# PaulTFLi/Machine-Learning-Replications

Measured on AMD Instinct MI355X. Metric: train_rows_per_sec, higher is better.
Workload: dtype fp32

## Files before the change

machine-learning-replications_amd/ops/csrc/svm_ws.hip:

```cpp
#include <type_traits>

#include "common.h"

namespace hfens {

struct WsProb {
  long long zoff;
  long long aoff;
  int l;
  int npos;
  double Cp, Cn;
  float ngl2e;
  int pad;
};

struct WsState {
  int done;
  int outer;
  long long inner;
  double gap;
  int nc;
  int nws;
  int nprev;
  int pad;
// ... 119 lines not shown
    if (pos ? a < C : a > 0) { su = -yg; ku = ws_key(su); }
    if (pos ? a > 0 : a < C) { sl = yg; kl = ws_key(sl); }
    X.keys[P.aoff + t] = ku;
    X.keys[X.n + P.aoff + t] = kl;
  }
  su = wave_max_f64_exact(su);
  sl = wave_max_f64_exact(sl);
  if ((threadIdx.x & 63) == 0) {
    if (su > -kWsInf) atomicMax(&X.gkey[2 * b], f64_okey(su));
    if (sl > -kWsInf) atomicMax(&X.gkey[2 * b + 1], f64_okey(sl));
  }
}

__global__ __launch_bounds__(256) void ws_init_kernel(const WsProb* __restrict__ probs, const float* __restrict__ zcat,
                                                      int F, float* __restrict__ zn, double* __restrict__ alpha,
                                                      double* __restrict__ G, WsState* __restrict__ states,
                                                      WsAux X) {
  const int b = blockIdx.y;
  const WsProb P = probs[b];
  const int t = blockIdx.x * blockDim.x + threadIdx.x;
  if (blockIdx.x * blockDim.x >= P.l) return;
  if (blockIdx.x == 0 && threadIdx.x == 0) states[b] = WsState{0, 0, 0, 0.0, 0, 0, 0, 0, 0, 0, 0, 0, 0, 0};
  const bool valid = t < P.l;
  if (valid) {
    const float* z = zcat + (P.zoff + t) * F;
    float s = 0.f;
    for (int k = 0; k < F; ++k) s = fmaf(z[k], z[k], s);
    zn[P.aoff + t] = s;
    alpha[P.aoff + t] = 0.0;
    G[P.aoff + t] = -1.0;
  }
  ws_publish_keys(P, b, t, valid, 0.0, -1.0, X);
}

constexpr size_t ws_sel_lds_bytes(int Q) { return 32 * 4 + 4096 * 4 + 1024 * 4 + (size_t)Q * 4; }

template <int M, typename Emit>
__device__ __forceinline__ int ws_pick_lists(const unsigned (&ku)[M], const unsigned (&kl)[M], int t0, int k_up,
                                             int k_low, int* shi, int* binfo, int* hist, Emit emit) {
  const int tid = threadIdx.x;
  for (int i = tid; i < 4096; i += kWsThreads) hist[i] = 0;
  if (tid < 8) binfo[tid] = 0;
  __syncthreads();
#pragma unroll
  for (int m = 0; m < M; ++m) {
    hist_add(hist, ku[m] != 0u, (int)(ku[m] >> 21));
    hist_add(hist, kl[m] != 0u, 2048 + (int)(kl[m] >> 21));
  }
  __syncthreads();
  ws_find_bin(hist, k_up, k_low, shi, binfo);
  __syncthreads();
  const unsigned bu1 = binfo[0], bl1 = binfo[2];
  const int au1 = binfo[1], al1 = binfo[3];
  for (int i = tid; i < 4096; i += kWsThreads) hist[i] = 0;
  __syncthreads();
#pragma unroll
  for (int m = 0; m < M; ++m) {
    hist_add(hist, ku[m] != 0u && (ku[m] >> 21) == bu1, (int)((ku[m] >> 10) & 2047));
    hist_add(hist, kl[m] != 0u && (kl[m] >> 21) == bl1, 2048 + (int)((kl[m] >> 10) & 2047));
  }
  __syncthreads();
  ws_find_bin(hist, k_up - au1, k_low - al1, shi, binfo + 4);
  __syncthreads();
  const unsigned Tu = (bu1 << 11) | (unsigned)binfo[4], Tl = (bl1 << 11) | (unsigned)binfo[6];
  const int need_u = k_up - au1 - binfo[5], need_l = k_low - al1 - binfo[7];
  unsigned selm = 0u;
  int base = 0;
#pragma unroll
  for (int side = 0; side < 2; ++side) {
    const unsigned T = side ? Tl : Tu;
    const int need = side ? need_l : need_u;
    int wt = 0;
#pragma unroll
    for (int m = 0; m < M; ++m) {
      const unsigned k = side ? kl[m] : ku[m];
      wt += __popcll(__ballot(k && (k >> 10) == T && !((selm >> m) & 1u)));
    }
    int ttot;
    int trank = wave_base(wt, shi, &ttot);
    unsigned pick = 0u;
    int ws_cnt = 0;
#pragma unroll
    for (int m = 0; m < M; ++m) {
      const unsigned k = side ? kl[m] : ku[m];
      const bool cand = k && !((selm >> m) & 1u);
      const bool tie = cand && (k >> 10) == T;
      const unsigned long long tb = __ballot(tie);
      const bool take = cand && ((k >> 10) > T || (tie && trank + __popcll(tb & lanes_below()) < need));
      trank += __popcll(tb);
      if (take) pick |= 1u << m;
      ws_cnt += __popcll(__ballot(take));
    }
    int stot;
    int pos = base + wave_base(ws_cnt, shi, &stot);
#pragma unroll
    for (int m = 0; m < M; ++m) {
      const bool take = (pick >> m) & 1u;
      const unsigned long long tb = __ballot(take);
      if (take) emit(pos + __popcll(tb & lanes_below()), t0 + 64 * m);
      pos += __popcll(tb);
    }
    selm |= pick;
    base += stot;
  }
  return base;
}

struct WsCand {
  int* idx;
  unsigned* ku;
  unsigned* kl;
  int ncand;
};
constexpr int kWsCandM = 8;
constexpr int kWsCandBlk = kWsCandM * kWsThreads;

template <int M, int Q, bool kWriteIdx, bool kCand = false>
__device__ __forceinline__ int ws_select_body(const WsProb& P, int b, WsState* S, int* __restrict__ wsidx,
                                              int* __restrict__ wsprev, double eps, int max_outer, const WsAux& X,
                                              int* shi, int* binfo, int* hist, unsigned* bm, int* widx,
                                              const WsCand& C = WsCand{nullptr, nullptr, nullptr, 0}) {
  const int nprev = S->nprev;
  const int tid = threadIdx.x;
  const int lane = tid & 63, wave = tid >> 6;
  const int L = kCand ? C.ncand : P.l;
  const int t0 = wave * 64 * M + lane;
  const long long c0 = __builtin_amdgcn_s_memtime();
  const unsigned long long gku = X.gkey[2 * b], gkl = X.gkey[2 * b + 1];
  const double Gmax = gku ? f64_from_okey(gku) : -kWsInf;
  const double Gmax2 = gkl ? f64_from_okey(gkl) : -kWsInf;
  const double gap = Gmax + Gmax2;
  unsigned ku[M], kl[M];
  int nu = 0, nl = 0;
#pragma unroll
  for (int m = 0; m < M; ++m) {
    const int t = t0 + 64 * m;
    if (kCand) {
      ku[m] = t < L ? C.ku[(size_t)b * C.ncand + t] : 0u;
      kl[m] = t < L ? C.kl[(size_t)b * C.ncand + t] : 0u;
    } else {
      ku[m] = t < L ? __builtin_nontemporal_load(X.keys + P.aoff + t) : 0u;
      kl[m] = t < L ? __builtin_nontemporal_load(X.keys + X.n + P.aoff + t) : 0u;
    }
  }
#pragma unroll
  for (int m = 0; m < M; ++m) {
    nu += __popcll(__ballot(ku[m] != 0u));
    nl += __popcll(__ballot(kl[m] != 0u));
  }
  if (!kCand)
    for (int i = tid; i < 1024; i += kWsThreads) bm[i] = 0;
  int n_up;
  wave_base(nu | (nl << 16), shi, &n_up);
  const int n_low = n_up >> 16;
  n_up &= 0xFFFF;
  if (!(gap >= eps) || S->outer >= max_outer || n_up == 0 || n_low == 0) {
    if (tid == 0) { S->done = 1; S->gap = gap; S->nc = 0; S->nws = 0; }
    return -1;
  }
  if (tid == 0) { X.gkey[2 * b] = 0ull; X.gkey[2 * b + 1] = 0ull; }
  const int k_up = min(Q / 4, n_up), k_low = min(Q / 4, n_low);
  const long long c0a = __builtin_amdgcn_s_memtime();
  const int nnew = ws_pick_lists<M>(ku, kl, t0, k_up, k_low, shi, binfo, hist, [&](int i, int p) {
    if (kCand) {
      widx[i] = C.idx[(size_t)b * C.ncand + p];
    } else {
      widx[i] = p;
      atomicOr(&bm[p >> 5], 1u << (p & 31));
    }
  });
  const long long c0b = __builtin_amdgcn_s_memtime();
  const long long c0c = c0b;
  __syncthreads();
  const int pv = tid < nprev ? wsprev[(size_t)b * (Q / 2) + tid] : -1;
  bool again = false;
  if (pv >= 0) {
    if (kCand) {
      for (int w = 0; w < nnew; ++w) again |= widx[w] == pv;
    } else {
      again = (bm[pv >> 5] >> (pv & 31)) & 1u;
    }
  }
  const bool keep = pv >= 0 && !again;
  const unsigned long long kb = __ballot(keep);
  int ktot;
  const int kpos = nnew + wave_base(__popcll(kb), shi, &ktot) + __popcll(kb & lanes_below());
  if (keep) widx[kpos] = pv;
  __syncthreads();
  const int nws = nnew + ktot;
  for (int w = tid; w < nnew; w += kWsThreads) wsprev[(size_t)b * (Q / 2) + w] = widx[w];
  if (kWriteIdx)
    for (int w = tid; w < nws; w += kWsThreads) wsidx[(size_t)b * Q + w] = widx[w];
  const long long c1 = __builtin_amdgcn_s_memtime();
  if (tid == 0) {
    S->cyc_select += c1 - c0;
    S->cyc_p0 += c0a - c0;
    S->cyc_p1 += c0b - c0a;
    S->cyc_p2 += c0c - c0b;
    S->nws = nws;
    S->nprev = nnew;
    S->gap = gap;
  }
  return nws;
}

template <int Q>
__global__ __launch_bounds__(kWsThreads) void ws_cand_kernel(const WsProb* __restrict__ probs,
                                                             const WsState* __restrict__ states, WsAux X, WsCand C) {
  constexpr int M = kWsCandM;
  constexpr int per = Q / 2;
  const int b = blockIdx.y, blk = blockIdx.x;
  if (states[b].done) return;
  const WsProb P = probs[b];
  const int tid = threadIdx.x;
  const int lane = tid & 63, wave = tid >> 6;
  const int beg = blk * kWsCandBlk;
  int* out_idx = C.idx + (size_t)b * C.ncand + (size_t)blk * per;
  unsigned* out_ku = C.ku + (size_t)b * C.ncand + (size_t)blk * per;
  unsigned* out_kl = C.kl + (size_t)b * C.ncand + (size_t)blk * per;
  __shared__ int shi[16], binfo[16];
  __shared__ int hist[4096];
  __shared__ int pick[per];
  const int t0 = wave * 64 * M + lane;
  unsigned ku[M], kl[M];
  int nu = 0, nl = 0;
#pragma unroll
  for (int m = 0; m < M; ++m) {
    const int t = beg + t0 + 64 * m;
    ku[m] = t < P.l ? __builtin_nontemporal_load(X.keys + P.aoff + t) : 0u;
    kl[m] = t < P.l ? __builtin_nontemporal_load(X.keys + X.n + P.aoff + t) : 0u;
  }
#pragma unroll
  for (int m = 0; m < M; ++m) {
    nu += __popcll(__ballot(ku[m] != 0u));
    nl += __popcll(__ballot(kl[m] != 0u));
  }
  int n_up;
  wave_base(nu | (nl << 16), shi, &n_up);
  const int n_low = n_up >> 16;
  n_up &= 0xFFFF;
  const int np = (n_up == 0 && n_low == 0) ? 0
                 : ws_pick_lists<M>(ku, kl, t0, min(Q / 4, n_up), min(Q / 4, n_low), shi, binfo, hist,
                                    [&](int i, int p) { pick[i] = beg + p; });
  __syncthreads();
  if (tid < per) {
    const int t = tid < np ? pick[tid] : -1;
    out_idx[tid] = t;
    out_ku[tid] = t >= 0 ? X.keys[P.aoff + t] : 0u;
    out_kl[tid] = t >= 0 ? X.keys[X.n + P.aoff + t] : 0u;
  }
}

template <int M, int Q>
__global__ __launch_bounds__(kWsThreads) void ws_select_kernel(
    const WsProb* __restrict__ probs, WsState* __restrict__ states, int* __restrict__ wsidx,
    int* __restrict__ wsprev, double eps, int max_outer, WsAux X) {
  const int b = blockIdx.x;
  WsState* S = states + b;
  if (S->done) return;
  const WsProb P = probs[b];
  extern __shared__ __attribute__((aligned(16))) unsigned char ws_lds[];
  int* shi = reinterpret_cast<int*>(ws_lds);
  int* binfo = shi + 16;
  int* hist = shi + 32;
  unsigned* bm = reinterpret_cast<unsigned*>(hist + 4096);
  int* widx = reinterpret_cast<int*>(bm + 1024);
  ws_select_body<M, Q, true>(P, b, S, wsidx, wsprev, eps, max_outer, X, shi, binfo, hist, bm, widx);
}

constexpr size_t ws_solve_lds_bytes(int Q, int FP) {
  return 64 * 4 + (size_t)Q * FP * 4 + (size_t)Q * 4 * 2 + (size_t)6 * Q * 4;
}

template <int FP, int Q, int TH>
__global__ __launch_bounds__(TH) void ws_solve_kernel(
    const WsProb* __restrict__ probs, WsState* __restrict__ states, const float* __restrict__ zcat, int F,
    const float* __restrict__ zn_all, double* __restrict__ alpha_all, const double* __restrict__ G_all,
    const int* __restrict__ wsidx, float* __restrict__ wsz, float* __restrict__ wsn, float* __restrict__ wdc,
    int Fp2, double eps, int max_inner, double inner_frac, long long* __restrict__ prof) {
  static_assert(Q % TH == 0 && (Q & (Q - 1)) == 0 && TH % 64 == 0 && TH <= 512, "whole slots per thread");
  static_assert(FP % 4 == 0, "z rows are read as float4");
  constexpr int SL = Q / TH;
  static_assert(SL % 2 == 0, "slots go in pairs (packed f32 fma)");
  constexpr int NW = TH / 64;
  constexpr unsigned kIdx = Q - 1;
  const int b = blockIdx.x;
  WsState* S = states + b;
  if (S->done) return;
  const WsProb P = probs[b];
  const int nws = S->nws;
  const int tid = threadIdx.x;
  const int lane = tid & 63, wave = tid >> 6;
  extern __shared__ __attribute__((aligned(16))) unsigned char ws_lds[];
  unsigned* red = reinterpret_cast<unsigned*>(ws_lds);
  float* zB = reinterpret_cast<float*>(ws_lds + 64 * 4);
  float* snB = zB + (size_t)Q * FP;
  int* widx = reinterpret_cast<int*>(snB + Q);
  float* gl = reinterpret_cast<float*>(widx + Q);
  float* al = gl + 2 * Q;
  float* kil = al + 2 * Q;
  const double* Gp = G_all + P.aoff;
  double* ap = alpha_all + P.aoff;
  const long long c1 = __builtin_amdgcn_s_memtime();
  {
    int wi[SL];
#pragma unroll
    for (int m = 0; m < SL; ++m) {
      const int s = tid + TH * m;
      wi[m] = s < nws ? wsidx[(size_t)b * Q + s] : -1;
    }
    float zv[SL][FP];
    float znv[SL];
#pragma unroll
    for (int m = 0; m < SL; ++m) {
      const float* zrow = zcat + (P.zoff + (wi[m] < 0 ? 0 : wi[m])) * F;
#pragma unroll
      for (int k = 0; k < FP; ++k) zv[m][k] = (wi[m] >= 0 && k < F) ? zrow[k] : 0.f;
      znv[m] = wi[m] >= 0 ? zn_all[P.aoff + wi[m]] : 0.f;
    }
#pragma unroll
    for (int m = 0; m < SL; ++m) {
      const int s = tid + TH * m;
      widx[s] = wi[m] < 0 ? 0 : wi[m];
      snB[s] = P.ngl2e * znv[m];
#pragma unroll
      for (int k = 0; k < FP; k += 4)
        *reinterpret_cast<f32x4*>(&zB[s * FP + k]) = f32x4{zv[m][k], zv[m][k + 1], zv[m][k + 2], zv[m][k + 3]};
    }
  }
  __syncthreads();
  const long long c2 = __builtin_amdgcn_s_memtime();
  const long long r2 = __builtin_amdgcn_s_memrealtime();
  bool valid[SL], pos[SL];
  int tt[SL];
  float y[SL], Cw[SL], a[SL], yg[SL], sn[SL], tu[SL], tl[SL];
  double a0[SL];
  f32x2 zp[SL / 2][FP];
#pragma unroll
  for (int m = 0; m < SL; ++m) {
    const int s = tid + TH * m;
    valid[m] = s < nws;
    tt[m] = valid[m] ? widx[s] : 0;
    pos[m] = tt[m] < P.npos;
    y[m] = pos[m] ? 1.f : -1.f;
    Cw[m] = (float)(pos[m] ? P.Cp : P.Cn);
    tu[m] = valid[m] ? (pos[m] ? Cw[m] : 0.f) : -INFINITY;
    tl[m] = valid[m] ? (pos[m] ? 0.f : Cw[m]) : -INFINITY;
    a0[m] = valid[m] ? ap[tt[m]] : 0.0;
    a[m] = (float)a0[m];
    yg[m] = valid[m] ? y[m] * (float)Gp[tt[m]] : 0.f;
    sn[m] = valid[m] ? snB[s] : 0.f;
#pragma unroll
    for (int k = 0; k < FP; k += 4) {
      const f32x4 v = valid[m] ? *reinterpret_cast<const f32x4*>(&zB[s * FP + k]) : f32x4{0.f, 0.f, 0.f, 0.f};
#pragma unroll
      for (int q = 0; q < 4; ++q) zp[m / 2][k + q][m & 1] = v[q];
    }
  }
  const float k2c = -2.f * P.ngl2e;
  const float Cpf = (float)P.Cp, Cnf = (float)P.Cn;
  auto krow = [&](int r, float (&out)[SL]) {
    f32x2 d[SL / 2];
#pragma unroll
    for (int h = 0; h < SL / 2; ++h) d[h] = f32x2{0.f, 0.f};
#pragma unroll
    for (int k = 0; k < FP; k += 4) {
      const f32x4 v = *reinterpret_cast<const f32x4*>(&zB[r * FP + k]);
#pragma unroll
      for (int q = 0; q < 4; ++q) {
#pragma unroll
        for (int h = 0; h < SL / 2; ++h) d[h] = __builtin_elementwise_fma(f32x2{v[q], v[q]}, zp[h][k + q], d[h]);
      }
    }
    const float snr = snB[r];
#pragma unroll
    for (int m = 0; m < SL; ++m)
      out[m] = __builtin_amdgcn_exp2f(fminf(fmaf(k2c, d[m / 2][m & 1], snr + sn[m]), 0.f));
  };
  auto red4 = [&](const unsigned* r) {
    unsigned x = 0u;
#pragma unroll
    for (int w = 0; w < NW; w += 4) {
      const uint4 v = *reinterpret_cast<const uint4*>(r + w);
      x = max(max(x, max(v.x, v.y)), max(v.z, v.w));
    }
    return x;
  };
  float tol_in = -1.f;
  const float epsf = (float)eps;
#ifdef HFENS_WS_STAMPS
  const bool pf = prof != nullptr;
  long long ph[6] = {0, 0, 0, 0, 0, 0};
  long long tp = pf ? __builtin_amdgcn_s_memtime() : 0;
#define WS_STAMP(k)                                         \
  if (pf) {                                                 \
    const long long tn = __builtin_amdgcn_s_memtime();      \
    ph[k] += tn - tp;                                       \
    tp = tn;                                                \
  }
#else
  const bool pf = false;
  long long ph[6] = {0, 0, 0, 0, 0, 0};
#define WS_STAMP(k)
#endif
  int it = 0;
  auto pair = [&](auto parc) -> bool {
    constexpr int par = decltype(parc)::value;
    float* glp = gl + par * Q;
    float* alp = al + par * Q;
    float* kip = kil + par * Q;
    unsigned* r1 = red + (0 * 2 + par) * NW;
    unsigned* r3 = red + (1 * 2 + par) * NW;
    unsigned* r2 = red + (2 * 2 + par) * NW;
    unsigned* r4 = red + (3 * 2 + par) * NW;
    unsigned k1 = 0u, k3 = 0u, k4 = 0u;
    bool low[SL];
#pragma unroll
    for (int m = 0; m < SL; ++m) {
      const unsigned s = (unsigned)(tid + TH * m);
      glp[s] = yg[m];
      alp[s] = a[m];
      const float ya = y[m] * a[m];
      const bool up = ya < tu[m];
      low[m] = -ya < tl[m];
      const unsigned um = 0u - (unsigned)up, lm = 0u - (unsigned)low[m];
      const unsigned kv = f32_okey(-yg[m]) & um;
      k4 = max(k4, kv);
      k1 = max(k1, ((kv & ~kIdx) | s) & um);
      k3 = max(k3, f32_okey(yg[m]) & lm);
    }
    k1 = wave_max_u32(k1);
    k3 = wave_max_u32(k3);
    k4 = wave_max_u32(k4);
    if (lane == 0) { r1[wave] = k1; r3[wave] = k3; r4[wave] = k4; }
    WS_STAMP(0)
    __syncthreads();
    const unsigned K1 = __builtin_amdgcn_readfirstlane(red4(r1));
    const unsigned K3 = __builtin_amdgcn_readfirstlane(red4(r3));
    const unsigned K4 = __builtin_amdgcn_readfirstlane(red4(r4));
    if (K1 == 0u || K3 == 0u) return false;
    const int i = (int)(K1 & kIdx);
    const float ygi = glp[i];
    const bool ipos = widx[i] < P.npos;
    const float yi = ipos ? 1.f : -1.f;
    const float Gi = yi * ygi;
    const float GmaxB = -ygi;
    const float lgap = f32_from_okey(K4) + f32_from_okey(K3);
    if (tol_in < 0.f) tol_in = fmaxf(0.9999f * epsf, (float)inner_frac * lgap);
    if (lgap < tol_in) return false;
    WS_STAMP(1)
    float Ki[SL];
    krow(i, Ki);
    unsigned k2 = 0u;
#pragma unroll
    for (int m = 0; m < SL; ++m) {
      const unsigned s = (unsigned)(tid + TH * m);
      kip[s] = Ki[m];
      const float gd = GmaxB + yg[m];
      const float q0 = 2.f - 2.f * Ki[m];
      const float quad = q0 <= 0.f ? 1e-12f : q0;
      const unsigned ok = 0u - (unsigned)(low[m] & (gd > 0.f));
      k2 = max(k2, ((f32_okey(gd * gd * __builtin_amdgcn_rcpf(quad)) & ~kIdx) | s) & ok);
    }
    k2 = wave_max_u32(k2);
    if (lane == 0) r2[wave] = k2;
    WS_STAMP(2)
    __syncthreads();
    const unsigned K2 = __builtin_amdgcn_readfirstlane(red4(r2));
    if (K2 == 0u) return false;
    const int j = (int)(K2 & kIdx);
    const float ai_old = alp[i], aj_old = alp[j];
    const float Kij = kip[j];
    const bool jpos = widx[j] < P.npos;
    const float yj = jpos ? 1.f : -1.f;
    const float Gj = yj * glp[j];
    const float Ci = ipos ? Cpf : Cnf, Cj = jpos ? Cpf : Cnf;
    WS_STAMP(3)
    const float q0 = 2.f - 2.f * Kij;
    const float rq = __builtin_amdgcn_rcpf(q0 <= 0.f ? 1e-12f : q0);
    float ao, bo, as, bs;
    {
      const float delta = (-Gi - Gj) * rq;
      const float diff = ai_old - aj_old;
      ao = ai_old + delta;
      bo = aj_old + delta;
      const bool c1 = (diff > 0.f) & (bo < 0.f), c2 = !(diff > 0.f) & (ao < 0.f);
      ao = c1 ? diff : (c2 ? 0.f : ao);
      bo = c1 ? 0.f : (c2 ? -diff : bo);
      const bool c3 = (diff > Ci - Cj) & (ao > Ci), c4 = !(diff > Ci - Cj) & (bo > Cj);
      ao = c3 ? Ci : (c4 ? Cj + diff : ao);
      bo = c3 ? Ci - diff : (c4 ? Cj : bo);
    }
    {
      const float delta = (Gi - Gj) * rq;
      const float sum = ai_old + aj_old;
      as = ai_old - delta;
      bs = aj_old + delta;
      const bool c1 = (sum > Ci) & (as > Ci), c2 = !(sum > Ci) & (bs < 0.f);
      as = c1 ? Ci : (c2 ? sum : as);
      bs = c1 ? sum - Ci : (c2 ? 0.f : bs);
      const bool c3 = (sum > Cj) & (bs > Cj), c4 = !(sum > Cj) & (as < 0.f);
      as = c3 ? sum - Cj : (c4 ? 0.f : as);
      bs = c3 ? Cj : (c4 ? sum : bs);
    }
    const bool opp = ipos != jpos;
    const float ai = opp ? ao : as, aj = opp ? bo : bs;
    const float ci = yi * (ai - ai_old), cj = yj * (aj - aj_old);
    WS_STAMP(4)
    float Kj[SL];
    krow(j, Kj);
#pragma unroll
    for (int m = 0; m < SL; ++m) {
      const int s = tid + TH * m;
      a[m] = s == i ? ai : (s == j ? aj : a[m]);
      yg[m] += fmaf(Ki[m], ci, Kj[m] * cj);
    }
    WS_STAMP(5)
    ++it;
    return true;
  };
  while (it < max_inner && pair(std::integral_constant<int, 0>{}) && it < max_inner &&
         pair(std::integral_constant<int, 1>{})) {
  }
#undef WS_STAMP
  if (pf && tid == 0) {
#pragma unroll
    for (int k = 0; k < 6; ++k) prof[(size_t)b * 6 + k] += ph[k];
  }
  int nc = 0;
#pragma unroll
  for (int m = 0; m < SL; ++m) {
    const int s = tid + TH * m;
    double anew = a0[m];
    if (valid[m] && a[m] != (float)a0[m]) {
      const double C = pos[m] ? P.Cp : P.Cn;
      anew = a[m] <= 0.f ? 0.0 : (a[m] >= Cw[m] ? C : a0[m] + ((double)a[m] - (double)(float)a0[m]));
      anew = fmin(fmax(anew, 0.0), C);
    }
    const bool ch = valid[m] && anew != a0[m];
    const unsigned long long cm = __ballot(ch);
    __syncthreads();
    if (lane == 0) red[wave] = (unsigned)__popcll(cm);
    __syncthreads();
    int wb = 0, tot = 0;
#pragma unroll
    for (int w = 0; w < NW; ++w) {
      const int v = (int)red[w];
      wb += w < wave ? v : 0;
      tot += v;
    }
    const int cpos = nc + wb + __popcll(cm & lanes_below());
    if (ch) {
      ap[tt[m]] = anew;
      for (int k = 0; k < Fp2; ++k) wsz[((size_t)b * Fp2 + k) * Q + cpos] = k < F ? zB[s * FP + k] : 0.f;
      wsn[(size_t)b * Q + cpos] = sn[m];
      wdc[(size_t)b * Q + cpos] = (float)((double)y[m] * (anew - a0[m]));
    }
    nc += tot;
  }
  const int ncp = (nc + 31) & ~31;
  for (int p = nc + tid; p < ncp; p += TH) {
    for (int k = 0; k < Fp2; ++k) wsz[((size_t)b * Fp2 + k) * Q + p] = 0.f;
    wsn[(size_t)b * Q + p] = 0.f;
    wdc[(size_t)b * Q + p] = 0.f;
  }
  const long long c3 = __builtin_amdgcn_s_memtime();
  const long long r3 = __builtin_amdgcn_s_memrealtime();
  if (tid == 0) {
    S->cyc_build += c2 - c1;
    S->cyc_inner += c3 - c2;
    S->cyc_p2 += r3 - r2;
    if (it == 0 || nc == 0) S->done = 1;
    S->nc = nc;
    S->outer += 1;
    S->inner += it;
  }
}

__device__ __forceinline__ unsigned sel4u(const unsigned (&v)[4], int m) {
  const unsigned m0 = 0u - (unsigned)(m == 0), m1 = 0u - (unsigned)(m == 1);
  const unsigned m2 = 0u - (unsigned)(m == 2), m3 = 0u - (unsigned)(m == 3);
  return (v[0] & m0) | (v[1] & m1) | (v[2] & m2) | (v[3] & m3);
}

constexpr int kKcQ = 256;
constexpr int kKcQP = kKcQ + 1;
constexpr int kKcTri = kKcQ * (kKcQ + 1) / 2;
constexpr size_t kc_zbuf_bytes(int KS) {
  return (size_t)2 * KS * kKcQP * 4 > (4096 + 1024) * 4 ? (size_t)2 * KS * kKcQP * 4 : (4096 + 1024) * 4;
}
constexpr size_t kc_lds_bytes(int KS) { return 128 + 2 * kKcQ * 4 + (kc_zbuf_bytes(KS) + 15) / 16 * 16 + (size_t)kKcTri * 4; }
static_assert(kc_lds_bytes(12) <= 163840, "the K-cached round must fit the CU's 160 KiB of LDS");

__device__ __forceinline__ int kc_rowstart(int r) { return r * kKcQ - ((r * (r - 1)) >> 1); }

__device__ __forceinline__ float sel4(const float (&v)[4], int m) {
  const unsigned u[4] = {__float_as_uint(v[0]), __float_as_uint(v[1]), __float_as_uint(v[2]), __float_as_uint(v[3])};
  return __uint_as_float(sel4u(u, m));
}
__device__ __forceinline__ int sel4(const int (&v)[4], int m) {
  const unsigned u[4] = {(unsigned)v[0], (unsigned)v[1], (unsigned)v[2], (unsigned)v[3]};
  return (int)sel4u(u, m);
}
__device__ __forceinline__ float rdlane_f(float v, int l) { return __int_as_float(__builtin_amdgcn_readlane(__float_as_int(v), l)); }

template <int M, int KS, bool kCand, bool kStamp = false>
__global__ __launch_bounds__(kWsThreads) void ws_kc_round_kernel(
    const WsProb* __restrict__ probs, WsState* __restrict__ states, const float* __restrict__ zcat, int F,
    const float* __restrict__ zn_all, double* __restrict__ alpha_all, const double* __restrict__ G_all,
    int* __restrict__ wsprev, float* __restrict__ wsz, float* __restrict__ wsn, float* __restrict__ wdc,
    int Fp2, double eps, int max_outer, int max_inner, double inner_frac, WsAux X, WsCand C,
    long long* __restrict__ prof = nullptr) {
  constexpr int Q = kKcQ;
  constexpr int SL = Q / 64;
  constexpr unsigned kIdx = Q - 1;
  static_assert(SL == 4, "sel4 assumes four slots per lane");
  const int b = blockIdx.x;
  WsState* S = states + b;
  if (S->done) return;
  const WsProb P = probs[b];
  const int tid = threadIdx.x;
  const int lane = tid & 63, wave = tid >> 6;
  extern __shared__ __attribute__((aligned(16))) unsigned char ws_lds[];
  int* shi = reinterpret_cast<int*>(ws_lds);
  int* binfo = shi + 16;
  int* widx = shi + 32;
  float* snB = reinterpret_cast<float*>(widx + Q);
  float* zbuf = snB + Q;
  int* hist = reinterpret_cast<int*>(zbuf);
  unsigned* bm = reinterpret_cast<unsigned*>(hist + 4096);
  float* tri = zbuf + (kc_zbuf_bytes(KS) + 15) / 16 * 4;
  const int nws = ws_select_body<M, Q, false, kCand>(P, b, S, nullptr, wsprev, eps, max_outer, X, shi, binfo,
                                                     hist, bm, widx, C);
  if (nws < 0) return;
  const long long c1 = __builtin_amdgcn_s_memtime();
  for (int e = tid; e < 2 * KS * Q; e += kWsThreads) {
    const int k = e / Q, s = e - k * Q;
    zbuf[k * kKcQP + s] = (s < nws && k < F) ? zcat[(P.zoff + widx[s]) * F + k] : 0.f;
  }
  if (tid < Q) snB[tid] = tid < nws ? P.ngl2e * zn_all[P.aoff + widx[tid]] : 0.f;
  __syncthreads();
  {
    const int r32 = lane & 31, hi = lane >> 5;
    const float k2 = -2.f * P.ngl2e;
    for (int t = wave; t < 36; t += kWsWaves) {
      int ta = 0, rem = t;
      while (rem >= 8 - ta) { rem -= 8 - ta; ++ta; }
      const int tb = ta + rem;
      f32x16 A = {0.f};
#pragma unroll
      for (int q = 0; q < KS; ++q) {
        const float* zr = zbuf + (2 * q + hi) * kKcQP;
        A = __builtin_amdgcn_mfma_f32_32x32x2f32(zr[ta * 32 + r32], zr[tb * 32 + r32], A, 0, 0, 0);
      }
      const int col = tb * 32 + r32;
      const float snc = snB[col];
#pragma unroll
      for (int r = 0; r < 16; ++r) {
        const int row = ta * 32 + 8 * (r >> 2) + 4 * hi + (r & 3);
        const float kv = __builtin_amdgcn_exp2f(fminf(fmaf(k2, A[r], snB[row] + snc), 0.f));
        if (row <= col) tri[kc_rowstart(row) + col - row] = kv;
      }
    }
  }
  __syncthreads();
  const long long c2 = __builtin_amdgcn_s_memtime();
  if (wave != 0) return;
  const double* Gp = G_all + P.aoff;
  double* ap = alpha_all + P.aoff;
  bool valid[SL], pos[SL];
  int tt[SL], rb[SL];
  float y[SL], Cw[SL], a[SL], yg[SL], tu[SL], tl[SL];
  double a0[SL];
#pragma unroll
  for (int m = 0; m < SL; ++m) {
    const int s = 64 * m + lane;
    valid[m] = s < nws;
    tt[m] = valid[m] ? widx[s] : 0;
    pos[m] = tt[m] < P.npos;
    y[m] = pos[m] ? 1.f : -1.f;
    Cw[m] = (float)(pos[m] ? P.Cp : P.Cn);
    tu[m] = valid[m] ? (pos[m] ? Cw[m] : 0.f) : -INFINITY;
    tl[m] = valid[m] ? (pos[m] ? 0.f : Cw[m]) : -INFINITY;
    a0[m] = valid[m] ? ap[tt[m]] : 0.0;
    a[m] = (float)a0[m];
    yg[m] = valid[m] ? y[m] * (float)Gp[tt[m]] : 0.f;
    rb[m] = kc_rowstart(s) - s;
  }
  auto krow = [&](int r, float (&out)[SL]) {
    const int ra = kc_rowstart(r) - r;
#pragma unroll
    for (int m = 0; m < SL; ++m) {
      const int s = 64 * m + lane;
      out[m] = tri[s >= r ? ra + s : rb[m] + r];
    }
  };
  const float Cpf = (float)P.Cp, Cnf = (float)P.Cn;
  const float epsf = (float)eps;
  float tol_in = -1.f;
  int it = 0;
  long long ph[5] = {0, 0, 0, 0, 0};
  long long tp = kStamp ? (long long)__builtin_amdgcn_s_memtime() : 0;
  auto stamp = [&](int k) {
    if constexpr (kStamp) {
      const long long tn = __builtin_amdgcn_s_memtime();
      ph[k] += tn - tp;
      tp = tn;
    }
  };
  while (it < max_inner) {
    unsigned k1 = 0u, k3 = 0u;
    bool low[SL];
#pragma unroll
    for (int m = 0; m < SL; ++m) {
      const unsigned s = (unsigned)(64 * m + lane);
      const float ya = y[m] * a[m];
      const bool up = ya < tu[m];
      low[m] = -ya < tl[m];
      const unsigned um = 0u - (unsigned)up, lm = 0u - (unsigned)low[m];
      k1 = max(k1, ((f32_okey(-yg[m]) & ~kIdx) | s) & um);
      k3 = max(k3, f32_okey(yg[m]) & lm);
    }
    const unsigned K1 = __builtin_amdgcn_readfirstlane(wave_max_u32(k1));
    const unsigned K3 = __builtin_amdgcn_readfirstlane(wave_max_u32(k3));
    stamp(0);
    if (K1 == 0u || K3 == 0u) break;
    const int i = (int)(K1 & kIdx), mi = i >> 6, li = i & 63;
    const float ygi = rdlane_f(sel4(yg, mi), li);
    const float ai_old = rdlane_f(sel4(a, mi), li);
    const bool ipos = __builtin_amdgcn_readlane(sel4(tt, mi), li) < P.npos;
    const float yi = ipos ? 1.f : -1.f;
    const float Gi = yi * ygi;
    const float GmaxB = -ygi;
    const float lgap = GmaxB + f32_from_okey(K3);
    if (tol_in < 0.f) tol_in = fmaxf(0.9999f * epsf, (float)inner_frac * lgap);
    if (lgap < tol_in) break;
    float Ki[SL];
    krow(i, Ki);
    stamp(1);
    unsigned k2 = 0u;
#pragma unroll
    for (int m = 0; m < SL; ++m) {
      const unsigned s = (unsigned)(64 * m + lane);
      const float gd = GmaxB + yg[m];
      const float q0 = 2.f - 2.f * Ki[m];
      const float quad = q0 <= 0.f ? 1e-12f : q0;
      const unsigned ok = 0u - (unsigned)(low[m] & (gd > 0.f));
      k2 = max(k2, ((f32_okey(gd * gd * __builtin_amdgcn_rcpf(quad)) & ~kIdx) | s) & ok);
    }
    const unsigned K2 = __builtin_amdgcn_readfirstlane(wave_max_u32(k2));
    stamp(2);
    if (K2 == 0u) break;
    const int j = (int)(K2 & kIdx), mj = j >> 6, lj = j & 63;
    float Kj[SL];
    krow(j, Kj);
    const float ygj = rdlane_f(sel4(yg, mj), lj);
    const float aj_old = rdlane_f(sel4(a, mj), lj);
    const float Kij = rdlane_f(sel4(Ki, mj), lj);
    const bool jpos = __builtin_amdgcn_readlane(sel4(tt, mj), lj) < P.npos;
    const float yj = jpos ? 1.f : -1.f;
    const float Gj = yj * ygj;
    const float Ci = ipos ? Cpf : Cnf, Cj = jpos ? Cpf : Cnf;
    const float q0 = 2.f - 2.f * Kij;
    const float rq = __builtin_amdgcn_rcpf(q0 <= 0.f ? 1e-12f : q0);
    float ao, bo, as, bs;
    {
      const float delta = (-Gi - Gj) * rq;
      const float diff = ai_old - aj_old;
      ao = ai_old + delta;
      bo = aj_old + delta;
      const bool c1 = (diff > 0.f) & (bo < 0.f), c2 = !(diff > 0.f) & (ao < 0.f);
      ao = c1 ? diff : (c2 ? 0.f : ao);
      bo = c1 ? 0.f : (c2 ? -diff : bo);
      const bool c3 = (diff > Ci - Cj) & (ao > Ci), c4 = !(diff > Ci - Cj) & (bo > Cj);
      ao = c3 ? Ci : (c4 ? Cj + diff : ao);
      bo = c3 ? Ci - diff : (c4 ? Cj : bo);
    }
    {
      const float delta = (Gi - Gj) * rq;
      const float sum = ai_old + aj_old;
      as = ai_old - delta;
      bs = aj_old + delta;
      const bool c1 = (sum > Ci) & (as > Ci), c2 = !(sum > Ci) & (bs < 0.f);
      as = c1 ? Ci : (c2 ? sum : as);
      bs = c1 ? sum - Ci : (c2 ? 0.f : bs);
      const bool c3 = (sum > Cj) & (bs > Cj), c4 = !(sum > Cj) & (as < 0.f);
      as = c3 ? sum - Cj : (c4 ? 0.f : as);
      bs = c3 ? Cj : (c4 ? sum : bs);
    }
    const bool opp = ipos != jpos;
    const float ai = opp ? ao : as, aj = opp ? bo : bs;
    const float ci = yi * (ai - ai_old), cj = yj * (aj - aj_old);
    stamp(3);
#pragma unroll
    for (int m = 0; m < SL; ++m) {
      const int s = 64 * m + lane;
      a[m] = s == i ? ai : (s == j ? aj : a[m]);
      yg[m] += fmaf(Ki[m], ci, Kj[m] * cj);
    }
    stamp(4);
    ++it;
  }
  if constexpr (kStamp) {
    if (lane == 0)
      for (int k = 0; k < 5; ++k) prof[(size_t)b * 6 + k] += ph[k];
  }
  int nc = 0;
#pragma unroll
  for (int m = 0; m < SL; ++m) {
    const int s = 64 * m + lane;
    double anew = a0[m];
    if (valid[m] && a[m] != (float)a0[m]) {
      const double C = pos[m] ? P.Cp : P.Cn;
      anew = a[m] <= 0.f ? 0.0 : (a[m] >= Cw[m] ? C : a0[m] + ((double)a[m] - (double)(float)a0[m]));
      anew = fmin(fmax(anew, 0.0), C);
    }
    const bool ch = valid[m] && anew != a0[m];
    const unsigned long long cm = __ballot(ch);
    const int cpos = nc + __popcll(cm & lanes_below());
    if (ch) {
      ap[tt[m]] = anew;
      for (int k = 0; k < Fp2; ++k) wsz[((size_t)b * Fp2 + k) * Q + cpos] = zbuf[k * kKcQP + s];
      wsn[(size_t)b * Q + cpos] = snB[s];
      wdc[(size_t)b * Q + cpos] = (float)((double)y[m] * (anew - a0[m]));
    }
    nc += __popcll(cm);
  }
  const int ncp = (nc + 31) & ~31;
  for (int p = nc + lane; p < ncp; p += 64) {
    for (int k = 0; k < Fp2; ++k) wsz[((size_t)b * Fp2 + k) * Q + p] = 0.f;
    wsn[(size_t)b * Q + p] = 0.f;
    wdc[(size_t)b * Q + p] = 0.f;
  }
  const long long c3 = __builtin_amdgcn_s_memtime();
  if (lane == 0) {
    S->cyc_build += c2 - c1;
    S->cyc_inner += c3 - c2;
    if (it == 0 || nc == 0) S->done = 1;
    S->nc = nc;
    S->outer += 1;
    S->inner += it;
  }
}

template <int KS>
__global__ __launch_bounds__(256) void ws_gupdate_kernel(const WsProb* __restrict__ probs,
                                                         const WsState* __restrict__ states,
                                                         const float* __restrict__ zcat, int F,
                                                         const float* __restrict__ zn_all,
                                                         const double* __restrict__ alpha_all,
                                                         double* __restrict__ G_all,
                                                         const float* __restrict__ wsz,
                                                         const float* __restrict__ wsn,
                                                         const float* __restrict__ wdc, int Fp2, int Q, WsAux X) {
  const int b = blockIdx.y;
  const int nc = states[b].nc;
  if (nc == 0) return;
  const WsProb P = probs[b];
  const int row_blk = blockIdx.x * 256;
// ... 459 lines not shown
```

Baseline: 623,700.

## Fuse working-set build loads, prefetch kernel rows early, batch compaction barriers

The working-set build now issues all global loads (index, z row, norm, alpha, gradient) in one pass and fills the per-thread register copies straight from those values, instead of staging through LDS and reading them back after a barrier. The kernel-row computation is split into a load phase and a compute phase, so the LDS reads of row i and row j are issued as soon as the index is known and overlap the remaining reductions and the clipping math. The final compaction computes all per-slot ballots first and uses a single pair of barriers with a wider reduction buffer, rather than two barriers per slot. This raises register pressure and relies on unconditional loads at index 0 for invalid slots.

```diff
diff --git a/machine-learning-replications_amd/ops/csrc/svm_ws.hip b/machine-learning-replications_amd/ops/csrc/svm_ws.hip
--- a/machine-learning-replications_amd/ops/csrc/svm_ws.hip
+++ b/machine-learning-replications_amd/ops/csrc/svm_ws.hip
@@ -445,77 +445,78 @@
   const double* Gp = G_all + P.aoff;
   double* ap = alpha_all + P.aoff;
   const long long c1 = __builtin_amdgcn_s_memtime();
-  {
-    int wi[SL];
-#pragma unroll
-    for (int m = 0; m < SL; ++m) {
-      const int s = tid + TH * m;
-      wi[m] = s < nws ? wsidx[(size_t)b * Q + s] : -1;
-    }
-    float zv[SL][FP];
-    float znv[SL];
-#pragma unroll
-    for (int m = 0; m < SL; ++m) {
-      const float* zrow = zcat + (P.zoff + (wi[m] < 0 ? 0 : wi[m])) * F;
-#pragma unroll
-      for (int k = 0; k < FP; ++k) zv[m][k] = (wi[m] >= 0 && k < F) ? zrow[k] : 0.f;
-      znv[m] = wi[m] >= 0 ? zn_all[P.aoff + wi[m]] : 0.f;
-    }
-#pragma unroll
-    for (int m = 0; m < SL; ++m) {
-      const int s = tid + TH * m;
-      widx[s] = wi[m] < 0 ? 0 : wi[m];
-      snB[s] = P.ngl2e * znv[m];
-#pragma unroll
-      for (int k = 0; k < FP; k += 4)
-        *reinterpret_cast<f32x4*>(&zB[s * FP + k]) = f32x4{zv[m][k], zv[m][k + 1], zv[m][k + 2], zv[m][k + 3]};
-    }
-  }
-  __syncthreads();
-  const long long c2 = __builtin_amdgcn_s_memtime();
-  const long long r2 = __builtin_amdgcn_s_memrealtime();
   bool valid[SL], pos[SL];
   int tt[SL];
   float y[SL], Cw[SL], a[SL], yg[SL], sn[SL], tu[SL], tl[SL];
   double a0[SL];
   f32x2 zp[SL / 2][FP];
-#pragma unroll
-  for (int m = 0; m < SL; ++m) {
-    const int s = tid + TH * m;
-    valid[m] = s < nws;
-    tt[m] = valid[m] ? widx[s] : 0;
-    pos[m] = tt[m] < P.npos;
-    y[m] = pos[m] ? 1.f : -1.f;
-    Cw[m] = (float)(pos[m] ? P.Cp : P.Cn);
-    tu[m] = valid[m] ? (pos[m] ? Cw[m] : 0.f) : -INFINITY;
-    tl[m] = valid[m] ? (pos[m] ? 0.f : Cw[m]) : -INFINITY;
-    a0[m] = valid[m] ? ap[tt[m]] : 0.0;
-    a[m] = (float)a0[m];
-    yg[m] = valid[m] ? y[m] * (float)Gp[tt[m]] : 0.f;
-    sn[m] = valid[m] ? snB[s] : 0.f;
-#pragma unroll
-    for (int k = 0; k < FP; k += 4) {
-      const f32x4 v = valid[m] ? *reinterpret_cast<const f32x4*>(&zB[s * FP + k]) : f32x4{0.f, 0.f, 0.f, 0.f};
-#pragma unroll
-      for (int q = 0; q < 4; ++q) zp[m / 2][k + q][m & 1] = v[q];
-    }
-  }
+  {
+#pragma unroll
+    for (int m = 0; m < SL; ++m) {
+      const int s = tid + TH * m;
+      valid[m] = s < nws;
+      const int w = wsidx[(size_t)b * Q + (valid[m] ? s : 0)];
+      tt[m] = valid[m] ? w : 0;
+    }
+    float zv[SL][FP];
+    float znv[SL];
+    double gv[SL];
+#pragma unroll
+    for (int m = 0; m < SL; ++m) {
+      const float* zrow = zcat + (P.zoff + tt[m]) * F;
+#pragma unroll
+      for (int k = 0; k < FP; ++k) zv[m][k] = zrow[k + 8 <= FP ? k : min(k, F - 1)];
+      znv[m] = zn_all[P.aoff + tt[m]];
+      a0[m] = ap[tt[m]];
+      gv[m] = Gp[tt[m]];
+    }
+#pragma unroll
+    for (int m = 0; m < SL; ++m) {
+      const int s = tid + TH * m;
+      widx[s] = tt[m];
+      const float sns = P.ngl2e * (valid[m] ? znv[m] : 0.f);
+      snB[s] = sns;
+      sn[m] = valid[m] ? sns : 0.f;
+#pragma unroll
+      for (int k = 0; k < FP; ++k) zv[m][k] = (valid[m] && k < F) ? zv[m][k] : 0.f;
+#pragma unroll
+      for (int k = 0; k < FP; k += 4)
+        *reinterpret_cast<f32x4*>(&zB[s * FP + k]) = f32x4{zv[m][k], zv[m][k + 1], zv[m][k + 2], zv[m][k + 3]};
+#pragma unroll
+      for (int k = 0; k < FP; ++k) zp[m / 2][k][m & 1] = zv[m][k];
+      pos[m] = tt[m] < P.npos;
+      y[m] = pos[m] ? 1.f : -1.f;
+      Cw[m] = (float)(pos[m] ? P.Cp : P.Cn);
+      tu[m] = valid[m] ? (pos[m] ? Cw[m] : 0.f) : -INFINITY;
+      tl[m] = valid[m] ? (pos[m] ? 0.f : Cw[m]) : -INFINITY;
+      a0[m] = valid[m] ? a0[m] : 0.0;
+      a[m] = (float)a0[m];
+      yg[m] = valid[m] ? y[m] * (float)gv[m] : 0.f;
+    }
+  }
+  __syncthreads();
+  const long long c2 = __builtin_amdgcn_s_memtime();
+  const long long r2 = __builtin_amdgcn_s_memrealtime();
   const float k2c = -2.f * P.ngl2e;
   const float Cpf = (float)P.Cp, Cnf = (float)P.Cn;
-  auto krow = [&](int r, float (&out)[SL]) {
+  auto krow_load = [&](int r, f32x4 (&v)[FP / 4], float& snr) {
+#pragma unroll
+    for (int k = 0; k < FP; k += 4) v[k / 4] = *reinterpret_cast<const f32x4*>(&zB[r * FP + k]);
+    snr = snB[r];
+  };
+  auto krow = [&](const f32x4 (&v)[FP / 4], float snr, float (&out)[SL]) {
     f32x2 d[SL / 2];
 #pragma unroll
     for (int h = 0; h < SL / 2; ++h) d[h] = f32x2{0.f, 0.f};
 #pragma unroll
     for (int k = 0; k < FP; k += 4) {
-      const f32x4 v = *reinterpret_cast<const f32x4*>(&zB[r * FP + k]);
 #pragma unroll
       for (int q = 0; q < 4; ++q) {
 #pragma unroll
-        for (int h = 0; h < SL / 2; ++h) d[h] = __builtin_elementwise_fma(f32x2{v[q], v[q]}, zp[h][k + q], d[h]);
+        for (int h = 0; h < SL / 2; ++h)
+          d[h] = __builtin_elementwise_fma(f32x2{v[k / 4][q], v[k / 4][q]}, zp[h][k + q], d[h]);
       }
     }
-    const float snr = snB[r];
 #pragma unroll
     for (int m = 0; m < SL; ++m)
       out[m] = __builtin_amdgcn_exp2f(fminf(fmaf(k2c, d[m / 2][m & 1], snr + sn[m]), 0.f));
@@ -579,10 +580,13 @@
     WS_STAMP(0)
     __syncthreads();
     const unsigned K1 = __builtin_amdgcn_readfirstlane(red4(r1));
+    const int i = (int)(K1 & kIdx);
+    f32x4 zr[FP / 4];
+    float snr;
+    krow_load(i, zr, snr);
     const unsigned K3 = __builtin_amdgcn_readfirstlane(red4(r3));
     const unsigned K4 = __builtin_amdgcn_readfirstlane(red4(r4));
     if (K1 == 0u || K3 == 0u) return false;
-    const int i = (int)(K1 & kIdx);
     const float ygi = glp[i];
     const bool ipos = widx[i] < P.npos;
     const float yi = ipos ? 1.f : -1.f;
@@ -593,7 +597,7 @@
     if (lgap < tol_in) return false;
     WS_STAMP(1)
     float Ki[SL];
-    krow(i, Ki);
+    krow(zr, snr, Ki);
     unsigned k2 = 0u;
 #pragma unroll
     for (int m = 0; m < SL; ++m) {
@@ -612,6 +616,7 @@
     const unsigned K2 = __builtin_amdgcn_readfirstlane(red4(r2));
     if (K2 == 0u) return false;
     const int j = (int)(K2 & kIdx);
+    krow_load(j, zr, snr);
     const float ai_old = alp[i], aj_old = alp[j];
     const float Kij = kip[j];
     const bool jpos = widx[j] < P.npos;
@@ -651,7 +656,7 @@
     const float ci = yi * (ai - ai_old), cj = yj * (aj - aj_old);
     WS_STAMP(4)
     float Kj[SL];
-    krow(j, Kj);
+    krow(zr, snr, Kj);
 #pragma unroll
     for (int m = 0; m < SL; ++m) {
       const int s = tid + TH * m;
@@ -670,34 +675,44 @@
 #pragma unroll
     for (int k = 0; k < 6; ++k) prof[(size_t)b * 6 + k] += ph[k];
   }
+  static_assert(SL * NW <= 64, "the per-(m, wave) counts share the reduction slots");
+  double anew[SL];
+  bool ch[SL];
+  unsigned long long cm[SL];
+#pragma unroll
+  for (int m = 0; m < SL; ++m) {
+    anew[m] = a0[m];
+    if (valid[m] && a[m] != (float)a0[m]) {
+      const double C = pos[m] ? P.Cp : P.Cn;
+      anew[m] = a[m] <= 0.f ? 0.0 : (a[m] >= Cw[m] ? C : a0[m] + ((double)a[m] - (double)(float)a0[m]));
+      anew[m] = fmin(fmax(anew[m], 0.0), C);
+    }
+    ch[m] = valid[m] && anew[m] != a0[m];
+    cm[m] = __ballot(ch[m]);
+  }
+  __syncthreads();
+  if (lane == 0) {
+#pragma unroll
+    for (int m = 0; m < SL; ++m) red[m * NW + wave] = (unsigned)__popcll(cm[m]);
+  }
+  __syncthreads();
   int nc = 0;
 #pragma unroll
   for (int m = 0; m < SL; ++m) {
     const int s = tid + TH * m;
-    double anew = a0[m];
-    if (valid[m] && a[m] != (float)a0[m]) {
-      const double C = pos[m] ? P.Cp : P.Cn;
-      anew = a[m] <= 0.f ? 0.0 : (a[m] >= Cw[m] ? C : a0[m] + ((double)a[m] - (double)(float)a0[m]));
-      anew = fmin(fmax(anew, 0.0), C);
-    }
-    const bool ch = valid[m] && anew != a0[m];
-    const unsigned long long cm = __ballot(ch);
-    __syncthreads();
-    if (lane == 0) red[wave] = (unsigned)__popcll(cm);
-    __syncthreads();
     int wb = 0, tot = 0;
 #pragma unroll
     for (int w = 0; w < NW; ++w) {
-      const int v = (int)red[w];
+      const int v = (int)red[m * NW + w];
       wb += w < wave ? v : 0;
       tot += v;
     }
-    const int cpos = nc + wb + __popcll(cm & lanes_below());
-    if (ch) {
-      ap[tt[m]] = anew;
+    const int cpos = nc + wb + __popcll(cm[m] & lanes_below());
+    if (ch[m]) {
+      ap[tt[m]] = anew[m];
       for (int k = 0; k < Fp2; ++k) wsz[((size_t)b * Fp2 + k) * Q + cpos] = k < F ? zB[s * FP + k] : 0.f;
       wsn[(size_t)b * Q + cpos] = sn[m];
-      wdc[(size_t)b * Q + cpos] = (float)((double)y[m] * (anew - a0[m]));
+      wdc[(size_t)b * Q + cpos] = (float)((double)y[m] * (anew[m] - a0[m]));
     }
     nc += tot;
   }
```

After: 635,700, median of 4. +1.9%, better.
